# gregspangenberg/shoulder

Measured on AMD Instinct MI355X. Metric: humerus meshes/s end-to-end (all 4 landmarks), higher is better.
Workload: dtype f64 geometry + bf16 UNet

## Files before the change

shoulder_amd/csrc/k_groove.h:

```cpp
#pragma once
#include "k_stages.h"

namespace sh {

#define SH_GSLOTS (SH_GROOVE_NROWS * SH_MAXPEAK)

__global__ void k_groove_rows(const double* __restrict__ itr_cs , const double* __restrict__ prox_zs,
                              const double* __restrict__ canal_axis_ct, int row0,
                              double* __restrict__ xraw, double* __restrict__ ptheta, int* __restrict__ npk,
                              double* __restrict__ r0, int* __restrict__ err, int B) {
  __shared__ double s_bufA[SH_MPROX], s_bufB[SH_MPROX];
  double* const s_r = s_bufA; double* const s_filt = s_bufA;
  double* const s_neg = s_bufB; double* const s_roll = s_bufB;
  __shared__ int s_cand[SH_PEAK_CAP];
  __shared__ Peak s_pk[SH_PEAK_CAP];
  __shared__ int s_pass[SH_PEAK_CAP];
  __shared__ int s_ncand;
  const int M = SH_MPROX;
  const int gid = blockIdx.x, lane = threadIdx.x;
  const int b = gid / SH_GROOVE_NROWS, i = gid % SH_GROOVE_NROWS;
  const double* row = itr_cs + ((size_t)b * SH_NPROX + row0 + i) * 2 * M;
  const double* zs = prox_zs + (size_t)b * SH_NPROX + row0;
  for (int k = lane; k < M; k += 64) s_r[k] = row[M + k];
  if (lane == 0) s_ncand = 0;
// ... 155 lines not shown
    const double z_scaled = zs[i] * sc + (0.0 - zmin * sc);
    const double* ax = canal_axis_ct + 6 * b;
    double cu[3] = {ax[0] - ax[3], ax[1] - ax[4], ax[2] - ax[5]};
    const double n = norm3(cu);
    cu[0] /= n; cu[1] /= n; cu[2] /= n;
    const double z = zs[i], th = s_th[k];
    const double rad = row[M + s_pidx[k]];
    const double px = rad * cos(th), py = rad * sin(th);
    const double dx = px - cu[0] * z, dy = py - cu[1] * z;
    double* X = xraw + ((size_t)b * SH_GSLOTS + (size_t)i * SH_MAXPEAK + k) * 9;
    X[0] = rad; X[1] = near; X[2] = next; X[3] = z_scaled; X[4] = s_pk[k].prominence; X[5] = s_pk[k].width;
    X[6] = s_pk[k].width_height; X[7] = sqrt(dx * dx + dy * dy); X[8] = (double)np_ / 7.0;
    ptheta[(size_t)b * SH_GSLOTS + (size_t)i * SH_MAXPEAK + k] = th;
    for (int q = 0; q < 9; ++q) if (X[q] != X[q]) atomicCAS(&err[b], 0, SH_ERR_GEOMETRY_DEV);
  }
  if (lane == 0) npk[gid] = np_;
  (void)B;
}

__global__ void __launch_bounds__(256)
k_groove_scale(const double* __restrict__ xraw, const int* __restrict__ npk, double* __restrict__ stats, int B,
               int* __restrict__ slots_out , int* __restrict__ nslot_out ,
               float* __restrict__ proba ) {
  __shared__ double col[5][SH_GSLOTS];
  __shared__ int slot[SH_GSLOTS];
  __shared__ int P_s;
  const int b = blockIdx.x, tid = threadIdx.x;
  const double* X = xraw + (size_t)b * SH_GSLOTS * 9;
  const int* np_ = npk + (size_t)b * SH_GROOVE_NROWS;
  __shared__ int s_cnt[SH_GROOVE_NROWS];
  for (int i = tid; i < SH_GROOVE_NROWS; i += 256) s_cnt[i] = np_[i];
  __syncthreads();
  for (int i = tid; i < SH_GROOVE_NROWS; i += 256) {
    int off = 0;
    for (int j = 0; j < i; ++j) off += s_cnt[j];
    const int n = s_cnt[i];
    for (int k = 0; k < n; ++k) slot[off + k] = i * SH_MAXPEAK + k;
    if (i == SH_GROOVE_NROWS - 1) P_s = off + n;
  }
  __syncthreads();
  const int P = P_s;
  for (int p = tid; p < P; p += 256) slots_out[(size_t)b * SH_GSLOTS + p] = slot[p];
  if (tid == 0) nslot_out[b] = P;
  for (int s = tid; s < SH_GSLOTS; s += 256)
    if (s % SH_MAXPEAK >= s_cnt[s / SH_MAXPEAK]) proba[(size_t)b * SH_GSLOTS + s] = -1.0f;
  for (int f0 = 0; f0 < 9; f0 += 5) {
    const int nf = f0 + 5 <= 9 ? 5 : 9 - f0;
    for (int q = tid; q < P * nf; q += 256) { const int p = q / nf, f = q - p * nf; col[f][p] = X[(size_t)slot[p] * 9 + f0 + f]; }
    __syncthreads();
    if (tid < nf) {
      const double* c = col[tid];
      double s = 0.0;
      int p = 0;
      for (; p + 8 <= P; p += 8) {
        double t8[8];
#pragma unroll
        for (int u = 0; u < 8; ++u) t8[u] = c[p + u];
#pragma unroll
        for (int u = 0; u < 8; ++u) s += t8[u];
      }
      for (; p < P; ++p) s += c[p];
      const double mean = P ? s / (double)P : 0.0;
      double v = 0.0;
      p = 0;
      for (; p + 8 <= P; p += 8) {
        double t8[8];
#pragma unroll
        for (int u = 0; u < 8; ++u) t8[u] = c[p + u];
#pragma unroll
        for (int u = 0; u < 8; ++u) { const double d = t8[u] - mean; v += d * d; }
      }
      for (; p < P; ++p) { double d = c[p] - mean; v += d * d; }
      const double var = P ? v / (double)P : 0.0;
      const double eps_ = 2.220446049250313e-16, nn = (double)P;
      const double ub = nn * eps_ * var + (nn * mean * eps_) * (nn * mean * eps_);
      double scale = var <= ub ? 1.0 : sqrt(var);
      stats[(size_t)b * 18 + f0 + tid] = mean;
      stats[(size_t)b * 18 + 9 + f0 + tid] = scale;
    }
    __syncthreads();
  }
}

__global__ void k_rfc_pack(const int* __restrict__ feat, const float* __restrict__ thr, const int* __restrict__ ti, const int* __restrict__ fi,
                           const float* __restrict__ lw, int4* __restrict__ nodes, int N) {
  const int i = blockIdx.x * blockDim.x + threadIdx.x;
  if (i >= N) return;
  const bool leaf = ti[i] < 0;
  nodes[i] = make_int4(feat[i], __float_as_int(leaf ? lw[i] : thr[i]), ti[i], fi[i]);
}

__global__ void __launch_bounds__(64)
k_groove_rfc(const double* __restrict__ xraw, const int* __restrict__ slots , const int* __restrict__ nslot , const double* __restrict__ stats,
             const int4* __restrict__ nodes, const int* __restrict__ roots, int n_trees,
             double* __restrict__ xs , float* __restrict__ proba, int B) {
  __shared__ double sx[9][64];
  const int tid = threadIdx.x;
  constexpr int WPB = (SH_GSLOTS + 63) / 64;
  const int b = blockIdx.x / WPB, p = (blockIdx.x - b * WPB) * 64 + tid;
  if (b >= B || p >= nslot[b]) return;
  const int gid = b * SH_GSLOTS + slots[(size_t)b * SH_GSLOTS + p];
  for (int f = 0; f < 9; ++f) {
    const double v = (xraw[(size_t)gid * 9 + f] - stats[(size_t)b * 18 + f]) / stats[(size_t)b * 18 + 9 + f];
    xs[(size_t)gid * 9 + f] = v;
    sx[f][tid] = v;
  }
  double acc = 0.0;
  for (int t = 0; t < n_trees; ++t) {
    int4 nd = nodes[roots[t]];
    while (nd.z >= 0) nd = nodes[(sx[nd.x][tid] <= (double)__int_as_float(nd.y)) ? nd.z : nd.w];
    acc += (double)__int_as_float(nd.y);
  }
  proba[gid] = (float)acc;
}

#define SH_KDE_TIE 1e-9
__device__ inline double groove_kde_wg(const double* __restrict__ ptheta, const float* __restrict__ proba, double* __restrict__ bg_theta,
                                       int* __restrict__ err, int b) {
  __shared__ double sel[SH_GSLOTS];
  __shared__ double dens[1024];
  __shared__ int nsel;
  __shared__ double wv[4];
  __shared__ int wi[4];
  __shared__ double s_bg;
  int tid = threadIdx.x;
  __shared__ int s_wc[4];
  if (tid == 0) nsel = 0;
  __syncthreads();
  for (int s0 = 0; s0 < SH_GSLOTS; s0 += 256) {
    const int s = s0 + tid;
    const bool keep = s < SH_GSLOTS && proba[(size_t)b * SH_GSLOTS + s] > 0.4f;
    const double val = keep ? ptheta[(size_t)b * SH_GSLOTS + s] : 0.0;
    const unsigned long long m = __ballot(keep);
    if ((tid & 63) == 0) s_wc[tid >> 6] = __popcll(m);
    __syncthreads();
    int pos = nsel + __popcll(m & ((1ull << (tid & 63)) - 1ull));
    for (int w = 0; w < (tid >> 6); ++w) pos += s_wc[w];
    if (keep) sel[pos] = val;
    __syncthreads();
    if (tid == 0) nsel += s_wc[0] + s_wc[1] + s_wc[2] + s_wc[3];
    __syncthreads();
  }
  const int n = nsel;
  if (n == 0) { if (tid == 0) { atomicCAS(&err[b], 0, SH_ERR_GEOMETRY_DEV); bg_theta[b] = 0.0; } return 0.0; }
  double best = -1.0;
  for (int j = tid; j < 1024; j += blockDim.x) {
    double t = linspace_at(-1.0 * M_PI, M_PI, 1024, j);
    double acc = 0.0;
    for (int i = 0; i < n; ++i) {
      double d = 1.0 - fabs(t - sel[i]);
      if (d > 0.0) acc += d;
    }
    dens[j] = acc;
    best = fmax(best, acc);
  }
  for (int off = 32; off > 0; off >>= 1) best = fmax(best, __shfl_down(best, off));
  if ((tid & 63) == 0) wv[tid >> 6] = best;
  __syncthreads();
  best = wv[0];
  for (int w = 1; w < (int)(blockDim.x >> 6); ++w) best = fmax(best, wv[w]);
  const double thr = best * (1.0 - SH_KDE_TIE);
  int bi = 0x7fffffff;
  for (int j = tid; j < 1024; j += blockDim.x)
    if (dens[j] >= thr) bi = min(bi, j);
  for (int off = 32; off > 0; off >>= 1) bi = min(bi, __shfl_down(bi, off));
  if ((tid & 63) == 0) wi[tid >> 6] = bi;
  __syncthreads();
  if (tid == 0) {
    for (int w = 1; w < (int)(blockDim.x >> 6); ++w) bi = min(bi, wi[w]);
    s_bg = linspace_at(-1.0 * M_PI, M_PI, 1024, bi);
    bg_theta[b] = s_bg;
  }
  __syncthreads();
  return s_bg;
}

__device__ inline void groove_localmin_row(const double* __restrict__ itr_cs, const double* __restrict__ r0, const double* __restrict__ prox_zs,
                                           const double* __restrict__ prox_centroids, double bg, int row0, double deg_window,
                                           int* __restrict__ local_idx, double* pts_obb, int b, int i) {
  const int gid = b * SH_GROOVE_NROWS + i;
  const double* row = itr_cs + ((size_t)b * SH_NPROX + row0 + i) * 2 * SH_MPROX;
  int ivar = (int)rint(deg_window / (360.0 / (double)SH_MPROX));
  if (ivar < 1) ivar = 1;
  int loc = groove_local_min(row, r0 + (size_t)gid * SH_MPROX, SH_MPROX, bg, ivar);
  local_idx[gid] = loc;
  int k = loc < 0 ? loc + SH_MPROX : loc;
  k = k < 0 ? 0 : (k >= SH_MPROX ? SH_MPROX - 1 : k);
  double t = row[k], r = row[SH_MPROX + k];
  const double* c = prox_centroids + 2 * ((size_t)b * SH_NPROX + row0 + i);
  double* p = pts_obb + (size_t)gid * 3;
  p[0] = r * cos(t) + c[0];
  p[1] = r * sin(t) + c[1];
  p[2] = prox_zs[(size_t)b * SH_NPROX + row0 + i] + 0.0;
}

__device__ inline void groove_axis_wave(const double* pts_obb, const double* __restrict__ T_obb, double* __restrict__ axis_ct,
// ... 34 lines not shown
```

shoulder_amd/csrc/k_stages.h:

```cpp
#pragma once
#include "k_slices.h"

namespace sh {

__global__ void k_synth_batch(const float* __restrict__ tv, const int* __restrict__ tf, long long V, long long F,
                              const double* __restrict__ T, float* __restrict__ verts, int* __restrict__ faces) {
  int b = blockIdx.y;
  const double* Tb = T + 16 * b;
  for (long long i = blockIdx.x * (long long)blockDim.x + threadIdx.x; i < V; i += (long long)gridDim.x * blockDim.x) {
    double o[3];
    xform_pt(Tb, (double)tv[3 * i], (double)tv[3 * i + 1], (double)tv[3 * i + 2], o);
    float* q = verts + 3 * (V * b + i);
    q[0] = (float)o[0]; q[1] = (float)o[1]; q[2] = (float)o[2];
  }
  for (long long i = blockIdx.x * (long long)blockDim.x + threadIdx.x; i < 3 * F; i += (long long)gridDim.x * blockDim.x)
    faces[3 * F * b + i] = tf[i];
}

__global__ void k_affine_f64(const double* __restrict__ T, const double* __restrict__ in, double* __restrict__ out,
                             const long long* __restrict__ off) {
  int b = blockIdx.y;
  const double* Tb = T + 16 * b;
  long long o0 = off[b], n = off[b + 1] - o0;
  for (long long i = blockIdx.x * (long long)blockDim.x + threadIdx.x; i < n; i += (long long)gridDim.x * blockDim.x) {
// ... 19 lines not shown
  const double ox = plane[0], oy = plane[1], oz = plane[2], nx = plane[3], ny = plane[4], nz = plane[5];
  for (long long fi = blockIdx.x * (long long)blockDim.x + threadIdx.x; fi < nf; fi += (long long)gridDim.x * blockDim.x) {
    int id[3] = {faces[3 * fi], faces[3 * fi + 1], faces[3 * fi + 2]};
    double P[3][3], d[3];
    int s[3];
    for (int k = 0; k < 3; ++k) {
      for (int q = 0; q < 3; ++q) P[k][q] = (double)verts[3 * (size_t)id[k] + q];
      d[k] = ((P[k][0] - ox) * nx + (P[k][1] - oy) * ny) + (P[k][2] - oz) * nz;
      s[k] = d[k] < -SH_SECTION_TOL ? -1 : 1;
    }
    if (s[0] == s[1] && s[1] == s[2]) continue;
    int dn = 0;
    for (int j = 0; j < 3; ++j) if (s[j] == 1 && s[(j + 1) % 3] == -1) dn = j;
    int a = dn, c = (dn + 1) % 3;
    int l = id[a] < id[c] ? a : c, h = id[a] < id[c] ? c : a;
    double t = d[l] / (d[l] - d[h]);
    int slot = atomicAdd(count, 1);
    if (slot < cap)
      for (int q = 0; q < 3; ++q) out[3 * (size_t)slot + q] = P[l][q] + t * (P[h][q] - P[l][q]);
  }
}

__device__ inline double wave_kth_smallest_nonneg(const double* v, int n, int k, unsigned* hist) {
  const int lane = threadIdx.x & 63;
  unsigned long long prefix = 0, mask = 0;
  for (int shift = 56; shift >= 0; shift -= 8) {
    for (int i = lane; i < 256; i += 64) hist[i] = 0;
    __syncthreads();
    for (int i = lane; i < n; i += 64) {
      const unsigned long long u = (unsigned long long)__double_as_longlong(v[i]);
      if ((u & mask) == prefix) atomicAdd(&hist[(u >> shift) & 255], 1u);
    }
    __syncthreads();
    const unsigned c0 = hist[4 * lane], c1 = hist[4 * lane + 1], c2 = hist[4 * lane + 2], c3 = hist[4 * lane + 3];
    const unsigned tot = c0 + c1 + c2 + c3;
    unsigned incl = tot;
    for (int off = 1; off < 64; off <<= 1) { unsigned o = __shfl_up(incl, off); if (lane >= off) incl += o; }
    const unsigned excl = incl - tot;
    if ((unsigned)k >= excl && (unsigned)k < incl) {
      unsigned r = (unsigned)k - excl, bin = 4 * lane;
      if (r >= c0) { r -= c0; ++bin; if (r >= c1) { r -= c1; ++bin; if (r >= c2) { r -= c2; ++bin; } } }
      hist[256] = bin; hist[257] = r;
    }
    __syncthreads();
    prefix |= (unsigned long long)hist[256] << shift;
    mask |= 0xffull << shift;
    k = (int)hist[257];
    __syncthreads();
  }
  return __longlong_as_double((long long)prefix);
}

template <bool BIG>
__global__ void __launch_bounds__(64)
k_neck(const double* __restrict__ areas, const double* __restrict__ zs, double* __restrict__ neck_z, int* __restrict__ neck_index, int B,
       double c0, double c1, double* __restrict__ gscratch ) {
  __shared__ double Ks[BIG ? 1 : SH_CPD_MAXN * SH_CPD_MAXN];
  __shared__ unsigned hist[258];
  int b = blockIdx.x, lane = threadIdx.x;
  int a, e;
  cutoff_range(SH_NFULL, c0, c1, &a, &e);
  int n = e - a;
  if (!BIG && n > SH_CPD_MAXN) n = SH_CPD_MAXN;
  double* K;
  if (BIG) K = gscratch + (size_t)b * SH_NFULL * SH_NFULL; else K = Ks;
  const double* x = areas + (size_t)b * SH_NFULL + a;
  for (int i = 0; i < n; ++i) {
    const int base = i * n - i * (i + 1) / 2 - (i + 1);
    for (int j = i + 1 + lane; j < n; j += 64) { double d = x[i] - x[j]; K[base + j] = d * d; }
  }
  __syncthreads();
  const int np_ = n * (n - 1) / 2;
  double med;
  __threadfence_block();
  if (np_ & 1) med = wave_kth_smallest_nonneg(K, np_, np_ / 2, hist);
  else { double lo = wave_kth_smallest_nonneg(K, np_, np_ / 2 - 1, hist); double hi = wave_kth_smallest_nonneg(K, np_, np_ / 2, hist); med = (lo + hi) / 2.0; }
  const double gamma = (med == 0.0) ? 1.0 : 1.0 / med;
  __syncthreads();
  for (int q = lane; q < n * n; q += 64) K[q] = cpd_kernel(x[q / n], x[q % n], gamma);
  __syncthreads();
  double best = 1e300;
  int bt = 0x7fffffff;
  for (int t = 2 + lane; t <= n - 2; t += 64) {
    double cst = cpd_cost(K, n, t);
    if (cst < best) { best = cst; bt = t; }
  }
  for (int off = 32; off > 0; off >>= 1) {
    double ob = __shfl_down(best, off);
    int ot = __shfl_down(bt, off);
    if (ob < best || (ob == best && ot < bt)) { best = ob; bt = ot; }
  }
  if (lane == 0) {
    neck_index[b] = bt;
    neck_z[b] = zs[(size_t)b * SH_NFULL + a + bt];
  }
}

__global__ void k_prox_obb(const double* __restrict__ area_scan , const double* __restrict__ scan_zs, const double* __restrict__ T_pre,
                           double* __restrict__ T_obb, int* __restrict__ flipped, double* __restrict__ cutoff , int* __restrict__ cutoff_idx ,
                           int* __restrict__ err, int B) {
  const int b = blockIdx.x * blockDim.x + threadIdx.x;
  if (b >= B) return;
  const double* A = area_scan + (size_t)b * SH_NPSCAN;
  int k = 0;
  for (int j = 1; j < SH_NPSCAN; ++j) if (A[j] > A[k]) k = j;
  const bool flip = scan_zs[(size_t)b * SH_NPSCAN + k] < 0;
  double ar[SH_NPSCAN], tmp[2 * SH_NPSCAN];
  for (int j = 0; j < SH_NPSCAN; ++j) ar[j] = flip ? A[SH_NPSCAN - 1 - j] : A[j];
  int lo, hi;
  if (prox_canal_range(ar, SH_NPSCAN, tmp, &lo, &hi) < 1) atomicCAS(&err[b], 0, SH_ERR_GEOMETRY_DEV);
  cutoff_idx[2 * b] = lo; cutoff_idx[2 * b + 1] = hi;
  cutoff[2 * b] = (double)lo / (double)SH_NPSCAN;
  cutoff[2 * b + 1] = (double)hi / (double)SH_NPSCAN;
  flipped[b] = flip ? 1 : 0;
  const double* Tp = T_pre + 16 * b;
  double* To = T_obb + 16 * b;
  for (int q = 0; q < 16; ++q) To[q] = Tp[q];
  if (flip) for (int q = 0; q < 4; ++q) { To[q] = -Tp[q]; To[8 + q] = -Tp[8 + q]; }
}

__device__ inline double wave_sum(double v) {
  for (int off = 32; off > 0; off >>= 1) v += __shfl_down(v, off);
  return __shfl(v, 0);
}

__device__ inline void wave_line_fit(const double* p, int n, int stride, double* mean, double* dir) {
  int lane = threadIdx.x & 63;
  double s[3] = {0, 0, 0};
  for (int i = lane; i < n; i += 64) { s[0] += p[(size_t)i * stride]; s[1] += p[(size_t)i * stride + 1]; s[2] += p[(size_t)i * stride + 2]; }
  for (int k = 0; k < 3; ++k) mean[k] = wave_sum(s[k]) / (double)n;
  double c[6] = {0, 0, 0, 0, 0, 0};
  for (int i = lane; i < n; i += 64) {
    double x = p[(size_t)i * stride] - mean[0], y = p[(size_t)i * stride + 1] - mean[1], z = p[(size_t)i * stride + 2] - mean[2];
    c[0] += x * x; c[1] += x * y; c[2] += x * z; c[3] += y * y; c[4] += y * z; c[5] += z * z;
  }
  for (int k = 0; k < 6; ++k) c[k] = wave_sum(c[k]);
  double C[9] = {c[0], c[1], c[2], c[1], c[3], c[4], c[2], c[4], c[5]};
  dominant_eigvec3(C, dir);
}

#define SH_CANAL_MAXPTS SH_NFULL
__global__ void k_canal(const double* __restrict__ centroids, const double* __restrict__ zs, const double* __restrict__ zb,
                        const double* __restrict__ T_obb, double c0, double c1, const double* __restrict__ cut ,
                        double* __restrict__ pts_obb, double* __restrict__ axis_obb, double* __restrict__ axis_ct, int* __restrict__ err) {
  int b = blockIdx.x, lane = threadIdx.x;
  if (cut) { c0 = cut[2 * b]; c1 = cut[2 * b + 1]; }
  int a, e;
  cutoff_range(SH_NFULL, c0, c1, &a, &e);
  int n = e - a;
  if (n > SH_CANAL_MAXPTS) n = SH_CANAL_MAXPTS;
  if (n < 2) { if (lane == 0) { atomicCAS(&err[b], 0, SH_ERR_GEOMETRY_DEV); for (int k = 0; k < 6; ++k) { axis_obb[6 * b + k] = 0; axis_ct[6 * b + k] = 0; } } return; }
  double* P = pts_obb + (size_t)b * SH_CANAL_MAXPTS * 3;
  for (int i = lane; i < n; i += 64) {
    P[3 * i] = centroids[2 * ((size_t)b * SH_NFULL + a + i)];
    P[3 * i + 1] = centroids[2 * ((size_t)b * SH_NFULL + a + i) + 1];
    P[3 * i + 2] = zs[(size_t)b * SH_NFULL + a + i];
  }
  __syncthreads();
  double mean[3], d[3];
  wave_line_fit(P, n, 3, mean, d);
  if (lane == 0) {
    if (d[2] < 0) { d[0] = -d[0]; d[1] = -d[1]; d[2] = -d[2]; }
    double z_length = fabs(zb[2 * b]) + fabs(zb[2 * b + 1]);
    double half = (z_length * ((c0 + c1) / 2.0)) / 2.0;
    double* A = axis_obb + 6 * b;
    for (int k = 0; k < 3; ++k) { A[k] = mean[k] + d[k] * half; A[3 + k] = mean[k] - d[k] * half; }
    double Ti[16];
// ... 8 lines not shown
```

shoulder_amd/csrc/sh_ctx.h:

```cpp
#pragma once
#include "../../include/shoulder_hip.h"

#include <hip/hip_runtime.h>

#include <algorithm>
#include <atomic>
#include <chrono>
#include <cmath>
#include <condition_variable>
#include <cstddef>
#include <cstdio>
#include <cstring>
#include <deque>
#include <functional>
#include <initializer_list>
#include <map>
#include <memory>
#include <mutex>
#include <string>
#include <thread>
#include <tuple>
#include <vector>

#include "sh_demand.h"
// ... 48 lines not shown
  int open_mode = SH_OPEN_ERROR;
  double open_gap = SH_OPEN_GAP_DEFAULT;
  int open_stats_run = SH_OPEN_ERROR;
  int end_cap = SH_ENDCAP;
  unsigned long long obb_gen = ~0ull;
  sh::HullCap hcap = {SH_HV, SH_HF, SH_HE};
  int obb_sil_need = 0;
  bool obb_nf_over = false;
  bool hull_force_host = false;
  std::vector<float> h_verts;
  bool h_verts_valid = false;
  float* h_kept = nullptr; long long h_kept_cap = 0;
  int* h_nkept = nullptr; int h_nkept_cap = 0;
  struct HullPts { const float* src = nullptr;
                   std::vector<long long> off;
                   std::vector<int> cnt; };
  HullPts hull_in;
  long long* h_koff = nullptr; int h_koff_cap = 0;
  struct StageSide {
    bool active = false, from_stl = false;
    int B = 0; long long sumV = 0, sumF = 0, maxV = 0, maxF = 0;
    std::vector<long long> voff, foff;
    void* h_src = nullptr; size_t h_src_cap = 0;
    int* h_flag = nullptr;
    size_t h_flag_cap = 0;
    float* h_kept = nullptr; long long h_kept_cap = 0;
    long long* h_koff = nullptr; int h_koff_cap = 0;
    HullPts pts;
    hipEvent_t ready_ev = nullptr;
    std::mutex m; std::condition_variable cv; bool meta_ready = true; int meta_rc = 0; std::string meta_err;
  } stg;
  int b0 = 0, Bwin = 0;
  struct HullStage { double* hv = nullptr; double* nr = nullptr; int* ed = nullptr; int* cnt = nullptr; int cap = 0; hipEvent_t ev = nullptr; bool used = false;
                     int pv = 4096, pf = 8192, pe = 12288; };
  HullStage hstage[2];
  int hslot = 0;
  struct Prepared {
    std::thread th; bool active = false; int slot = 0, B = 0, rc = SH_OK, bad_mesh = -1; unsigned long long gen = 0;
    double d2h_ms = 0, hull_ms = 0; std::string err;
    bool uploaded = false;
    bool staged = false;
  } prep;
  hipEvent_t obb_done_ev = nullptr;
  struct Ticket { hipEvent_t ev = nullptr; char* status = nullptr ; int cap = 0, B = 0; bool pending = false; sh_landmarks* host_out = nullptr;
                  uint32_t mask = 0; sh_landmarks* out_arg = nullptr; bool dev_hull = false; unsigned long long gen = 0; size_t rec = sizeof(sh_landmarks); int rows = 0; };
  Ticket tickets[2];
  int t_head = 0, t_tail = 0, n_pending = 0;
  hipStream_t out_stream = nullptr;
  bool overlap = false;
  unsigned long long batch_gen = 0;
  uint32_t rec_mask = 0;
  unsigned long long rec_gen = ~0ull, resect_gen = ~0ull;
  int resect_P = 0;
  unsigned long long canal_gen = ~0ull;
  sh_canal_grid canal_grid = {0.0, 0.0, 0, 0};
  unsigned long long resect_seq = 0, canal_seq = 0;
  unsigned long long seat_resect_seq = ~0ull, stem_resect_seq = ~0ull, stem_canal_seq = ~0ull;
  int seat_K = 0, stem_K = 0;
  hipStream_t copy_stream = nullptr;
  hipEvent_t stl_counted_ev = nullptr;
  hipStream_t side_stream = nullptr;
  hipEvent_t side_fork_ev = nullptr, side_join_ev = nullptr;
  struct Switches {
    int window = 0;
    bool obb_prune = true;
    bool slice_merge = true;
    bool hull_prefilter = true;
    bool debug = false;
  } sw;
  struct Unet {
    bool reference = false;
    bool turn = false;
    hipEvent_t done_ev = nullptr;
    int num_cus = 0;
    int ticket_next = 0;
    std::map<std::tuple<int, int, int>, std::pair<int, int>> tk_tabs;
    int tk_tab_used = 0;
    bool zero_page_ready = false;
    bool packtab_ready = false;
    bool packed_x3 = false;
    int packed_kind = -1;
  } unet;
  bool packed_rfc = false;
  int timing = 0;
  std::vector<std::tuple<std::string, hipEvent_t, hipEvent_t>> pending;
  std::map<std::string, KTimer> timers;
};

#define HIPCHK(ctx, call)                                                                   \
  do {                                                                                      \
    hipError_t e_ = (call);                                                                 \
    if (e_ != hipSuccess) {                                                                 \
      (ctx)->err = std::string(#call) + ": " + hipGetErrorString(e_);                       \
      return SH_ERR_HIP;                                                                    \
    }                                                                                       \
  } while (0)

#define HIPCHK_TXT(errtxt, call) do { hipError_t e_ = (call); if (e_ != hipSuccess) { *(errtxt) = std::string(#call) + ": " + hipGetErrorString(e_); return SH_ERR_HIP; } } while (0)

struct WindowScope {
  sh_ctx* c; int b0, Bwin;
  WindowScope(sh_ctx* c_, int nb0, int nBwin) : c(c_), b0(c_->b0), Bwin(c_->Bwin) { c->b0 = nb0; c->Bwin = nBwin; }
  ~WindowScope() { c->b0 = b0; c->Bwin = Bwin; }
  WindowScope(const WindowScope&) = delete; WindowScope& operator=(const WindowScope&) = delete;
};

struct StreamScope {
  sh_ctx* c; hipStream_t saved;
  StreamScope(sh_ctx* c_, hipStream_t s) : c(c_), saved(c_->stream) { c->stream = s; }
  ~StreamScope() { c->stream = saved; }
  StreamScope(const StreamScope&) = delete; StreamScope& operator=(const StreamScope&) = delete;
};

static inline void params_changed(sh_ctx* c) { c->unet.packed_kind = -1; c->unet.packed_x3 = false; c->packed_rfc = false; }

static inline int fail(sh_ctx* c, int code, const std::string& msg) {
  if (c) c->err = msg;
  return code;
}

static inline int ensure(sh_ctx* c, const char* name, size_t bytes, int elem, void** out = nullptr) {
  Buf& b = c->bufs[name];
  if (b.bytes < bytes || b.p == nullptr) {
    if (b.p) (void)hipFree(b.p);
    b.p = nullptr;
    hipError_t e = hipMalloc(&b.p, bytes ? bytes : 16);
    if (e != hipSuccess) {
      c->err = std::string("hipMalloc(") + name + "): " + hipGetErrorString(e);
      b.bytes = 0;
      return SH_ERR_NOMEM;
    }
    b.bytes = bytes;
  }
  b.elem = elem;
  if (out) *out = b.p;
  return SH_OK;
}

template <typename T>
static inline T* buf(sh_ctx* c, const char* name) {
  auto it = c->bufs.find(name);
  if (it == c->bufs.end() || !it->second.p) return nullptr;
  return (T*)((char*)it->second.p + (size_t)c->b0 * it->second.per_mesh);
}

struct HullRec { double *hv, *normals; int *edges, *nv, *nf, *ne; };
static inline HullRec hull_rec(sh_ctx* c) {
  return {buf<double>(c, "hull.hv"), buf<double>(c, "hull.normals"), buf<int>(c, "hull.edges"), buf<int>(c, "hull.nv"), buf<int>(c, "hull.nf"), buf<int>(c, "hull.ne")};
}

#define ENS_(name, bytes, elem, per_mesh_)                                          \
  do {                                                                              \
    if ((rc = ensure(c, name, (size_t)(bytes), elem)) != SH_OK) return rc;          \
    c->bufs[name].per_mesh = (per_mesh_);                                           \
  } while (0)
#define ENS(name, bytes, elem) ENS_(name, bytes, elem, (size_t)(bytes) / (size_t)c->B)
#define ENS_SHARED(name, bytes, elem) ENS_(name, bytes, elem, 0)
template <typename T> constexpr int elem_of() { return sizeof(T) <= 8 ? (int)sizeof(T) : 1; }

static inline bool timed_launch(const sh_ctx* c, const char* name) {
  return c->timing == 1 || (c->timing == 2 && name[0] == 'u' && name[1] == 'n' && name[2] == 'e' && name[3] == 't' && name[4] == '.');
}

#define LAUNCH_FN(ctx, name, call)                                                           \
  do {                                                                                      \
    hipEvent_t e0_ = nullptr, e1_ = nullptr;                                                \
// ... 41 lines not shown
```

shoulder_amd/csrc/sh_scalar.h:

```cpp
#pragma once
#include "sh_common.h"

namespace sh {

#define SH_CPD_MAXN 64
SH_HD double kth_smallest(double* a, int n, int k) {
  int lo = 0, hi = n - 1;
  while (lo < hi) {
    double p = a[(lo + hi) >> 1];
    int i = lo, j = hi;
    while (i <= j) {
      while (a[i] < p) ++i;
      while (a[j] > p) --j;
      if (i <= j) { double t = a[i]; a[i] = a[j]; a[j] = t; ++i; --j; }
    }
    if (k <= j) hi = j; else if (k >= i) lo = i; else break;
  }
  return a[k];
}

SH_HD double cpd_gamma(const double* x, int n, double* pd) {
  int np_ = n * (n - 1) / 2;
  int c = 0;
  for (int i = 0; i < n; ++i)
    for (int j = i + 1; j < n; ++j) { double d = x[i] - x[j]; pd[c++] = d * d; }
  double med;
  if (np_ & 1) med = kth_smallest(pd, np_, np_ / 2);
  else { double a = kth_smallest(pd, np_, np_ / 2 - 1); double b = kth_smallest(pd, np_, np_ / 2); med = (a + b) / 2.0; }
  return (med == 0.0) ? 1.0 : 1.0 / med;
}
SH_HD double cpd_kernel(double xi, double xj, double gamma) {
  double d = xi - xj;
  double v = d * d * gamma;
  v = v < 1e-2 ? 1e-2 : (v > 1e2 ? 1e2 : v);
  return exp(-v);
}
SH_HD double cpd_cost(const double* K, int n, int t) {
  double d0 = 0, s0 = 0, d1 = 0, s1 = 0;
  for (int i = 0; i < t; ++i) { d0 += K[i * n + i]; for (int j = 0; j < t; ++j) s0 += K[i * n + j]; }
  for (int i = t; i < n; ++i) { d1 += K[i * n + i]; for (int j = t; j < n; ++j) s1 += K[i * n + j]; }
  return (d0 - s0 / (double)t) + (d1 - s1 / (double)(n - t));
}
SH_HD int cpd_one_bkp(const double* x, int n, double* scratch) {
  const int min_size = 2;
  double* K = scratch + n * (n - 1) / 2;
  double gamma = cpd_gamma(x, n, scratch);
  for (int i = 0; i < n; ++i)
    for (int j = 0; j < n; ++j) K[i * n + j] = cpd_kernel(x[i], x[j], gamma);
  int best_t = -1;
  double best = 1e300;
  for (int t = min_size; t <= n - min_size; ++t) {
    double cst = cpd_cost(K, n, t);
    if (cst < best) { best = cst; best_t = t; }
  }
  return best_t;
}

SH_HD int prox_canal_range(const double* area, int n, double* tmp, int* lo, int* hi) {
  double* sm = tmp;
  double* g = tmp + n;
  for (int i = 1; i + 1 < n; ++i) sm[i] = ((area[i - 1] + area[i]) + area[i + 1]) / 3.0;
  sm[0] = ((5.0 * area[0] + 2.0 * area[1]) - area[2]) / 6.0;
  sm[n - 1] = ((5.0 * area[n - 1] + 2.0 * area[n - 2]) - area[n - 3]) / 6.0;
  g[0] = sm[1] - sm[0];
  g[n - 1] = sm[n - 1] - sm[n - 2];
  for (int i = 1; i + 1 < n; ++i) g[i] = (sm[i + 1] - sm[i - 1]) / 2.0;
  int best_a = 0, best_len = 0, a = -1;
  for (int i = 0; i <= n; ++i) {
    const bool in = i < n && g[i] < 10.0;
    if (in && a < 0) a = i;
    if (!in && a >= 0) { if (i - a > best_len) { best_len = i - a; best_a = a; } a = -1; }
  }
  *lo = best_a; *hi = best_len > 0 ? best_a + best_len - 1 : best_a;
  return best_len;
}

SH_HD double circle_residual_at(const double* xy, int n, double cx, double cy, double* g, double* H) {
  double sr = 0, sux = 0, suy = 0;
  for (int i = 0; i < n; ++i) {
    double dx = xy[2 * i] - cx, dy = xy[2 * i + 1] - cy;
    double r = sqrt(dx * dx + dy * dy);
    sr += r; sux += dx / r; suy += dy / r;
  }
  double rm = sr / n, mux = sux / n, muy = suy / n;
  double f2 = 0;
  if (g) { g[0] = g[1] = 0; H[0] = H[1] = H[2] = 0; }
  for (int i = 0; i < n; ++i) {
    double dx = xy[2 * i] - cx, dy = xy[2 * i + 1] - cy;
    double r = sqrt(dx * dx + dy * dy);
    double f = r - rm;
    f2 += f * f;
    if (g) {
      double jx = -(dx / r - mux), jy = -(dy / r - muy);
      g[0] += jx * f; g[1] += jy * f;
      H[0] += jx * jx; H[1] += jx * jy; H[2] += jy * jy;
    }
  }
  return f2;
}

SH_HD double circle_fit_residual(const double* xy, int n, double* cx_out = nullptr, double* cy_out = nullptr) {
  double cx = 0, cy = 0;
  for (int i = 0; i < n; ++i) { cx += xy[2 * i]; cy += xy[2 * i + 1]; }
  cx /= n; cy /= n;
  double lam = 1e-3, g[2], H[3];
  double f2 = circle_residual_at(xy, n, cx, cy, g, H);
  for (int it = 0; it < 200; ++it) {
    double a = H[0] * (1 + lam), b = H[1], d = H[2] * (1 + lam);
    double det = a * d - b * b;
    if (det == 0) break;
    double sx = -(d * g[0] - b * g[1]) / det, sy = -(-b * g[0] + a * g[1]) / det;
    double g2[2], H2[3];
    double f2n = circle_residual_at(xy, n, cx + sx, cy + sy, g2, H2);
    if (f2n <= f2) {
      cx += sx; cy += sy;
      bool done = (fabs(sx) + fabs(sy)) < 1e-13 * (1.0 + fabs(cx) + fabs(cy));
      f2 = f2n; g[0] = g2[0]; g[1] = g2[1]; H[0] = H2[0]; H[1] = H2[1]; H[2] = H2[2];
      lam *= 0.2;
      if (done) break;
    } else {
      lam *= 10.0;
      if (lam > 1e12) break;
    }
// ... 758 lines not shown
```

shoulder_amd/csrc/shoulder_hip.hip:

```cpp
#include "sh_ctx.h"

#include "k_slices.h"
#include "k_ovf.h"
#include "k_open.h"
#include "k_stages.h"
#include "k_groove.h"
#include "k_anp.h"
#include "k_stl.h"
#include "k_clip.h"
#include "k_resect.h"
#include "k_headfit.h"
#include "k_seat.h"
#include "k_stem.h"
#include "k_plan.h"
#include "k_te.h"
#include "k_obb.h"
#include "sh_hull.h"

#include <sched.h>

using namespace sh;

struct FillList { void* p[6]; unsigned long long n[6]; unsigned v[6]; };
__global__ void k_fill_list(FillList L) {
// ... 1333 lines not shown
  if (!c->obb_done_ev) HIPCHK(c, hipEventCreateWithFlags(&c->obb_done_ev, hipEventDisableTiming));
  HIPCHK(c, hipEventRecord(c->obb_done_ev, c->stream));
  if (c->params.bone_kind == SH_BONE_PROXIMAL) {
    dim3 gv((unsigned)std::min<long long>((c->maxV + 255) / 256, 1024), (unsigned)B);
    LAUNCH(c, "k_transform_verts", k_transform_verts, gv, dim3(256), v.verts, v.voff, v.obb_T_pre, v.verts_obb, v.zb_enc);
    w->bounds_cleared = false;
    int rc2;
    if ((rc2 = run_slice_set(c, v, SPEC_POBB)) != SH_OK) return rc2;
    LAUNCH(c, "k_prox_obb", k_prox_obb, dim3((B + 63) / 64), dim3(64), v.set[SET_POBB].area_total, v.set[SET_POBB].zs, v.obb_T_pre,
           v.obb_transform, v.flipped, v.pobb_cutoff, v.pobb_cutoff_idx, v.err, B);
    c->obb_injected = true;
    return SH_OK;
  }
  dim3 g((unsigned)std::min<long long>((c->maxF + 255) / 256, 1024), (unsigned)B);
  LAUNCH(c, "k_obb_end_points", k_obb_end_points, g, dim3(256), v.verts, v.faces, v.voff, v.foff, v.obb_T_pre, v.obb_zb_pre, v.obb_endpts, v.obb_endcnt, c->end_cap);
  LAUNCH(c, "k_obb_ends", k_obb_ends, dim3(B), dim3(128), v.obb_endpts, v.obb_endcnt, v.obb_T_pre, v.obb_resid, v.obb_transform, v.flipped, v.err, B, c->end_cap,
         v.ovf_ctr + SH_CTR_END_NEED);
  c->obb_injected = true;
  return SH_OK;
}

static int run_te_rows(sh_ctx* c, const WinView& v) {
  const int B = v.B;
  const SliceSetView& distal = v.set[SET_DISTAL];
  OvfPools OP; OvfSet OS;
  { int orc; if ((orc = ovf_pools(c, &OP)) != SH_OK || (orc = ovf_set(c, "distal", SH_NDIST, &OS)) != SH_OK) return orc; }
  LAUNCH(c, "k_te_rows", k_te_rows<SH_SMALLSEG>, dim3(B * SH_TE_NROWS), dim3(64), distal.ring, distal.ring_n, v.te_rects, B, (const long long*)OS.roff);
  LAUNCH(c, "k_te_rows_large", k_te_rows<SH_MAXSEG>, dim3(B * SH_TE_NROWS), dim3(64), distal.ring, distal.ring_n, v.te_rects, B, (const long long*)OS.roff);
  if (c->ovf_none_gen != c->batch_gen) LAUNCH(c, "k_te_rows_huge", k_te_rows_huge, dim3(64), dim3(64), OP, OS, (const int*)distal.ring_n, v.te_rects);
  LAUNCH(c, "k_te_ends", k_te_ends, dim3(B), dim3(64), distal.ring, distal.ring_n, v.te_rects, distal.zs, v.obb_transform, v.te_ends_ct, v.te_row, v.err, B, OP, OS);
  return SH_OK;
}

static int stage_frame(sh_ctx* c, const WinView& v, uint32_t mask, const WinState& w) {
  const int B = v.B;
  if (!w.bounds_cleared && (mask & (SH_STAGE_OBB | SH_STAGE_FULL | SH_STAGE_ANP)))
    FILL(c, {v.zb_enc, (size_t)B * 16, 0xFF}, {v.anp_mm_enc, (size_t)B * 16, 0xFF});
  if (mask & (SH_STAGE_OBB | SH_STAGE_FULL)) {
    dim3 g((unsigned)std::min<long long>((c->maxV + 255) / 256, 1024), (unsigned)B);
    LAUNCH(c, "k_transform_verts", k_transform_verts, g, dim3(256), v.verts, v.voff, v.obb_transform, v.verts_obb, v.zb_enc);
    if (!(mask & SH_STAGE_FULL))
      LAUNCH(c, "k_decode_bounds", k_decode_bounds, dim3((2 * B + 63) / 64), dim3(64), v.zb_enc, v.z_bounds, B);
  }
  return SH_OK;
}

static int fork_side(sh_ctx* c) {
  if (!c->side_stream) HIPCHK(c, hipStreamCreateWithFlags(&c->side_stream, hipStreamNonBlocking));
  if (!c->side_fork_ev) { HIPCHK(c, hipEventCreateWithFlags(&c->side_fork_ev, hipEventDisableTiming)); HIPCHK(c, hipEventCreateWithFlags(&c->side_join_ev, hipEventDisableTiming)); }
  HIPCHK(c, hipEventRecord(c->side_fork_ev, c->stream));
  HIPCHK(c, hipStreamWaitEvent(c->side_stream, c->side_fork_ev, 0));
  return SH_OK;
}

static int stage_distal(sh_ctx* c, const WinView& v, uint32_t mask, bool merged, bool side, WinState* w) {
  int rc;
  if (side && (rc = fork_side(c)) != SH_OK) return rc;
  {
    StreamScope on(c, side ? c->side_stream : c->stream);
    rc = merged ? SH_OK : run_slice_set(c, v, spec_distal(false));
    const bool te_inline = !side && (mask & SH_STAGE_ANP);
    if (rc == SH_OK && (side || te_inline) && (mask & SH_STAGE_TE)) { rc = run_te_rows(c, v); w->te_rows_done = rc == SH_OK; }
  }
  if (side && rc == SH_OK) { HIPCHK(c, hipEventRecord(c->side_join_ev, c->side_stream)); w->side_pending = true; }
  return rc;
}

static int stage_neck(sh_ctx* c, const WinView& v, bool with_prox) {
  const bool prox = c->params.bone_kind == SH_BONE_PROXIMAL;
  LAUNCH(c, "k_neck", prox ? k_neck<true> : k_neck<false>, dim3(v.B), dim3(64), v.set[SET_FULL].areas, v.set[SET_FULL].zs, v.neck_z, v.neck_index, v.B,
         prox ? 0.2 : 0.70, 0.99, prox ? v.neck_gram : (double*)nullptr);
  if (!with_prox) return run_slice_set(c, v, SPEC_NECKC);
  const SliceSpec sp[2] = {SPEC_NECKC, SPEC_PROX};
  return run_slice_sets(c, v, sp, 2);
}

static int stage_canal(sh_ctx* c, const WinView& v) {
  LAUNCH(c, "k_canal", k_canal, dim3(v.B), dim3(64), v.set[SET_FULL].centroids, v.set[SET_FULL].zs, v.z_bounds, v.obb_transform, c->params.canal_cutoff[0],
         c->params.canal_cutoff[1], c->params.bone_kind == SH_BONE_PROXIMAL ? v.pobb_cutoff : (const double*)nullptr,
         v.canal_points_obb, v.canal_axis_obb, v.canal_axis_ct, v.err);
  return SH_OK;
}

static int stage_groove(sh_ctx* c, const WinView& v, uint32_t mask) {
  const int B = v.B;
  int rc;
  if (!c->have_rfc) return fail(c, SH_ERR_STATE, "sh_run: groove stage needs sh_load_rfc first");
  int ga, gb;
  cutoff_range(SH_NPROX, c->params.groove_cutoff[0], c->params.groove_cutoff[1], &ga, &gb);
  if (!(mask & SH_STAGE_PROXIMAL) && !(c->rs_gen == c->batch_gen && (c->rs_all || (ga >= c->rs_cs_lo && gb <= c->rs_cs_hi))))
    return fail(c, SH_ERR_STATE, "sh_run: SH_STAGE_GROOVE without SH_STAGE_PROXIMAL, and the proximal slices of this batch were not made for this groove_cutoff (run SH_STAGE_PROXIMAL again)");
  const char* pp = buf<char>(c, "params") + c->unet_floats * 4;
  const size_t N = c->h_feat.size();
  const int* feat = (const int*)pp; const float* thr = (const float*)(pp + N * 4); const int* ti = (const int*)(pp + N * 8);
  const int* fi = (const int*)(pp + N * 12); const float* lw = (const float*)(pp + N * 16); const int* roots = (const int*)(pp + N * 20);
  const double* prox_zs = v.set[SET_PROX].zs;
  LAUNCH(c, "k_groove_rows", k_groove_rows, dim3(B * SH_GROOVE_NROWS), dim3(64), v.prox_itr_centered_start, prox_zs, v.canal_axis_ct, ga, v.groove_xraw,
         v.groove_ptheta, v.groove_npk, v.groove_r0, v.err, B);
  LAUNCH(c, "k_groove_scale", k_groove_scale, dim3(B), dim3(256), v.groove_xraw, v.groove_npk, v.groove_stats, B, v.groove_slots, v.groove_nslot, v.groove_proba);
  if ((rc = ensure(c, "rfc.nodes", N * 16, 4)) != SH_OK) return rc;
  int4* nodes = (int4*)c->bufs["rfc.nodes"].p;
  if (!c->packed_rfc) {
    LAUNCH(c, "k_rfc_pack", k_rfc_pack, dim3((unsigned)((N + 255) / 256)), dim3(256), feat, thr, ti, fi, lw, nodes, (int)N);
    c->packed_rfc = true;
  }
  LAUNCH(c, "k_groove_rfc", k_groove_rfc, dim3((unsigned)(B * ((SH_GSLOTS + 63) / 64))), dim3(64), v.groove_xraw, v.groove_slots, v.groove_nslot,
         v.groove_stats, nodes, roots, c->rfc_trees, v.groove_xs, v.groove_proba, B);
  LAUNCH(c, "k_groove_tail", k_groove_tail, dim3(B), dim3(256), v.groove_ptheta, v.groove_proba, v.groove_bg_theta, v.err,
         v.prox_itr_centered_start, v.groove_r0, prox_zs, v.set[SET_PROX].centroids, ga, c->params.groove_deg_window,
         v.groove_local_idx, v.groove_points_obb, v.obb_transform, v.groove_axis_ct, v.groove_points_ct);
  return SH_OK;
}

static int stage_anp(sh_ctx* c, const WinView& v) {
  const int B = v.B;
  int rc;
  if (!c->have_unet) return fail(c, SH_ERR_STATE, "sh_run: anatomic-neck stage needs sh_load_unet first");
  LAUNCH(c, "k_anp_rows", k_anp_rows, dim3(B * SH_ANP_ROWS), dim3(64), v.prox_itr_start, v.groove_bg_theta, v.anp_raw, v.anp_t01, v.anp_roll, B,
         v.anp_mm_enc);
  const bool scale_in_net = plan_level0_fused(c->params.unet_dtype, c->unet.reference, c->unet_base, c->unet_depth, SH_ANP_ROWS, SH_MPROX);
  if (!scale_in_net || c->keep_products) LAUNCH(c, "k_anp_scale", k_anp_scale, dim3(64, B), dim3(256), v.anp_raw, v.anp_mm_enc, v.anp_image);
  if ((rc = unet_turn_enter(c)) != SH_OK) return rc;
  rc = unet_dispatch(c, {v.anp_image, scale_in_net ? v.anp_raw : nullptr, scale_in_net ? v.anp_mm_enc : nullptr, v.anp_logits}, B, SH_ANP_ROWS, SH_MPROX);
  (void)unet_turn_leave(c);
  if (rc != SH_OK) return rc;
  const double* prox_zs = v.set[SET_PROX].zs;
  LAUNCH(c, "k_anp_edge_count", k_anp_edge_count, dim3(SH_ANP_ROWS / 8, B), dim3(512), v.anp_logits, v.anp_rowcnt, v.anp_maskbits);
  LAUNCH(c, "k_anp_edges", k_anp_edges, dim3(SH_ANP_ROWS / 8, B), dim3(512), v.anp_maskbits, v.anp_raw, v.anp_t01, v.anp_roll, prox_zs, v.anp_rowcnt,
         v.anp_points_obb, v.anp_counts, v.err);
  LAUNCH(c, "k_anp_plane", k_anp_plane, dim3(B), dim3(256), v.anp_points_obb, v.anp_counts, v.anp_plane, v.err, v.anp_ray_t);
  LAUNCH(c, "k_rays_hit", k_rays_hit, dim3(SH_RAY_CHUNKS, B), dim3(256), v.verts_obb, v.faces, v.voff, v.foff, v.anp_plane, v.anp_ray_t);
  return SH_OK;
}

static int stage_tail(sh_ctx* c, const WinView& v, uint32_t mask) {
  const int B = v.B;
  const bool prox = c->params.bone_kind == SH_BONE_PROXIMAL;
  const uint32_t need = SH_STAGE_GROOVE | SH_STAGE_ANP | SH_STAGE_CSYS | (prox ? 0u : (uint32_t)SH_STAGE_TE);
  const bool metrics = (mask & need) == need;
  if (metrics)
    LAUNCH(c, "k_sphere_partial", k_sphere_partial, dim3(SH_SPH_PARTS, B), dim3(256), v.anp_maskbits, v.anp_raw, v.anp_t01, v.anp_roll, v.set[SET_PROX].zs,
           v.anp_plane, v.metrics_partial);
  PackArgs A{};
  A.lm = v.landmarks; A.T_obb = v.obb_transform; A.zb = v.z_bounds; A.neck_z = v.neck_z;
  A.neck_index = v.neck_index; A.flipped = v.flipped; A.canal_axis_ct = v.canal_axis_ct; A.te_axis_ct = v.te_axis_ct;
  A.groove_axis_ct = v.groove_axis_ct; A.bg_theta = v.groove_bg_theta; A.groove_pts_ct = v.groove_points_ct;
  A.plane = v.anp_plane; A.axes_obb = v.anp_axes_obb; A.anp_pts_obb = v.anp_points_obb; A.anp_counts = v.anp_counts;
  A.err = v.err; A.mask = mask; A.B = B; A.bone_kind = (int)c->params.bone_kind;
  A.canal_cut = prox ? v.pobb_cutoff : (const double*)nullptr;
  A.cc0 = c->params.canal_cutoff[0]; A.cc1 = c->params.canal_cutoff[1];
  A.ray_t = v.anp_ray_t; A.te_ends_ct = v.te_ends_ct; A.sphere_partial = v.metrics_partial; A.metrics = metrics ? 1 : 0;
  LAUNCH(c, "k_tail", k_tail, dim3(B), dim3(256), A);
  return SH_OK;
}

static int stage_apply(sh_ctx* c, const WinView& v) {
  dim3 g((unsigned)std::min<long long>((c->maxV + 255) / 256, 1024), (unsigned)v.B);
  LAUNCH(c, "k_apply_csys", k_apply_csys, g, dim3(256), v.landmarks, v.verts, v.voff, v.verts_csys);
  return SH_OK;
}

static int run_window(sh_ctx* c, uint32_t mask, int prepared_slot, int redo_nf = 0) {
  auto has = [mask](uint32_t stages) { return (mask & stages) != 0; };
  int rc;
  WinView v = win_view(c);
  WinState w;
  if (has(SH_STAGE_OBB) && (rc = run_obb(c, v, &w, prepared_slot, redo_nf)) != SH_OK) return rc;
  if ((rc = stage_frame(c, v, mask, w)) != SH_OK) return rc;
  const bool transformed = has(SH_STAGE_OBB | SH_STAGE_FULL);
  const bool merge_env = c->sw.slice_merge;
  const bool can_fork = has(SH_STAGE_DISTAL) && c->ovf_none_gen == c->batch_gen && c->timing != 1 && redo_nf == 0;
  const bool side = can_fork && v.B <= 16;
  const bool merge_fd = merge_env && has(SH_STAGE_FULL) && has(SH_STAGE_DISTAL) && !side;
  if (merge_fd) {
    const SliceSpec sp[2] = {spec_full(transformed), spec_distal(transformed)};
    if ((rc = run_slice_sets(c, v, sp, 2)) != SH_OK) return rc;
  } else if (has(SH_STAGE_FULL)) {
    if ((rc = run_slice_set(c, v, spec_full(transformed))) != SH_OK) return rc;
  }
  if (has(SH_STAGE_DISTAL) && (rc = stage_distal(c, v, mask, merge_fd, side, &w)) != SH_OK) return rc;
  const bool merge_np = merge_env && has(SH_STAGE_NECK) && has(SH_STAGE_PROXIMAL);
  if (has(SH_STAGE_NECK) && (rc = stage_neck(c, v, merge_np)) != SH_OK) return rc;
  if (has(SH_STAGE_CANAL) && (rc = stage_canal(c, v)) != SH_OK) return rc;
  if (has(SH_STAGE_PROXIMAL) && !merge_np && (rc = run_slice_set(c, v, SPEC_PROX)) != SH_OK) return rc;
  if (has(SH_STAGE_GROOVE) && (rc = stage_groove(c, v, mask)) != SH_OK) return rc;
  if (has(SH_STAGE_ANP) && (rc = stage_anp(c, v)) != SH_OK) return rc;
  if (w.side_pending) { HIPCHK(c, hipStreamWaitEvent(c->stream, c->side_join_ev, 0)); w.side_pending = false; }
  if (has(SH_STAGE_TE) && !w.te_rows_done && (rc = run_te_rows(c, v)) != SH_OK) return rc;
  if ((rc = stage_tail(c, v, mask)) != SH_OK) return rc;
  if (has(SH_STAGE_APPLY) && (rc = stage_apply(c, v)) != SH_OK) return rc;
// ... 805 lines not shown
```

Before: 9278.

## Stage random-forest trees in LDS with BFS layout and double buffering

Random-forest inference now reorders each tree breadth-first on the host so its nodes sit contiguously with tree-relative child indices. It runs 256-thread blocks that stage each tree (up to 1024 nodes) in shared memory, double-buffered so the next tree's load overlaps the current walk. This replaces scattered global-memory node fetches with LDS reads, at the cost of a per-tree block barrier and more LDS per block. Separately, the neck CPD cost loop now uses an unrolled blocked row-sum helper.

```diff
diff --git a/shoulder_amd/csrc/k_groove.h b/shoulder_amd/csrc/k_groove.h
--- a/shoulder_amd/csrc/k_groove.h
+++ b/shoulder_amd/csrc/k_groove.h
@@ -261,36 +261,75 @@
   }
 }
 
-__global__ void k_rfc_pack(const int* __restrict__ feat, const float* __restrict__ thr, const int* __restrict__ ti, const int* __restrict__ fi,
-                           const float* __restrict__ lw, int4* __restrict__ nodes, int N) {
-  const int i = blockIdx.x * blockDim.x + threadIdx.x;
-  if (i >= N) return;
-  const bool leaf = ti[i] < 0;
-  nodes[i] = make_int4(feat[i], __float_as_int(leaf ? lw[i] : thr[i]), ti[i], fi[i]);
-}
-
-__global__ void __launch_bounds__(64)
+#define SH_RFC_LDS_NODES 1024
+__global__ void k_rfc_pack(const int* __restrict__ feat, const float* __restrict__ thr, const float* __restrict__ lw,
+                           const int* __restrict__ src, const int* __restrict__ lt, const int* __restrict__ lf, int4* __restrict__ nodes, int Np) {
+  const int q = blockIdx.x * blockDim.x + threadIdx.x;
+  if (q >= Np) return;
+  const int i = src[q];
+  const bool leaf = lt[q] < 0;
+  nodes[q] = make_int4(feat[i], __float_as_int(leaf ? lw[i] : thr[i]), lt[q], lf[q]);
+}
+
+typedef int rfc_node_t __attribute__((ext_vector_type(4)));
+
+template <typename NodePtr>
+__device__ inline double rfc_walk_tree(NodePtr T, const double (*sx)[256], int tid) {
+  int4 nd = T[0];
+  asm volatile("" : "+v"(nd.x), "+v"(nd.y), "+v"(nd.z), "+v"(nd.w));
+  while (nd.z >= 0) {
+    nd = T[(sx[nd.x][tid] <= (double)__int_as_float(nd.y)) ? nd.z : nd.w];
+    asm volatile("" : "+v"(nd.x), "+v"(nd.y), "+v"(nd.z), "+v"(nd.w));
+  }
+  return (double)__int_as_float(nd.y);
+}
+
+__global__ void __launch_bounds__(256)
 k_groove_rfc(const double* __restrict__ xraw, const int* __restrict__ slots , const int* __restrict__ nslot , const double* __restrict__ stats,
-             const int4* __restrict__ nodes, const int* __restrict__ roots, int n_trees,
+             const int4* __restrict__ nodes, const int2* __restrict__ trees , int n_trees,
              double* __restrict__ xs , float* __restrict__ proba, int B) {
-  __shared__ double sx[9][64];
+  __shared__ double sx[9][256];
+  __shared__ int4 s_tree[2][SH_RFC_LDS_NODES];
+  constexpr int NR = SH_RFC_LDS_NODES / 256;
   const int tid = threadIdx.x;
-  constexpr int WPB = (SH_GSLOTS + 63) / 64;
-  const int b = blockIdx.x / WPB, p = (blockIdx.x - b * WPB) * 64 + tid;
-  if (b >= B || p >= nslot[b]) return;
-  const int gid = b * SH_GSLOTS + slots[(size_t)b * SH_GSLOTS + p];
-  for (int f = 0; f < 9; ++f) {
-    const double v = (xraw[(size_t)gid * 9 + f] - stats[(size_t)b * 18 + f]) / stats[(size_t)b * 18 + 9 + f];
-    xs[(size_t)gid * 9 + f] = v;
-    sx[f][tid] = v;
-  }
+  constexpr int WPB = (SH_GSLOTS + 255) / 256;
+  const int b = blockIdx.x / WPB, p0 = (blockIdx.x - b * WPB) * 256;
+  if (b >= B) return;
+  const int ns = nslot[b];
+  if (p0 >= ns) return;
+  const bool live = p0 + tid < ns;
+  int gid = 0;
+  if (live) {
+    gid = b * SH_GSLOTS + slots[(size_t)b * SH_GSLOTS + p0 + tid];
+    for (int f = 0; f < 9; ++f) {
+      const double v = (xraw[(size_t)gid * 9 + f] - stats[(size_t)b * 18 + f]) / stats[(size_t)b * 18 + 9 + f];
+      xs[(size_t)gid * 9 + f] = v;
+      sx[f][tid] = v;
+    }
+  }
+  int2 cur = trees[0];
+  if (cur.y <= SH_RFC_LDS_NODES)
+    for (int k = tid; k < cur.y; k += 256) s_tree[0][k] = nodes[cur.x + k];
+  __syncthreads();
   double acc = 0.0;
   for (int t = 0; t < n_trees; ++t) {
-    int4 nd = nodes[roots[t]];
-    while (nd.z >= 0) nd = nodes[(sx[nd.x][tid] <= (double)__int_as_float(nd.y)) ? nd.z : nd.w];
-    acc += (double)__int_as_float(nd.y);
-  }
-  proba[gid] = (float)acc;
+    const bool more = t + 1 < n_trees;
+    const int2 nxt = more ? trees[t + 1] : make_int2(0, 0);
+    const bool stage = more && nxt.y <= SH_RFC_LDS_NODES;
+    rfc_node_t r[NR] = {};
+    if (stage) {
+#pragma unroll
+      for (int u = 0; u < NR; ++u) if (tid + 256 * u < nxt.y) r[u] = ((const rfc_node_t*)nodes)[nxt.x + tid + 256 * u];
+    }
+    if (live) acc += cur.y <= SH_RFC_LDS_NODES ? rfc_walk_tree((const int4*)s_tree[t & 1], sx, tid) : rfc_walk_tree(nodes + cur.x, sx, tid);
+    if (stage) {
+#pragma unroll
+      for (int u = 0; u < NR; ++u) if (tid + 256 * u < nxt.y) ((rfc_node_t*)s_tree[(t + 1) & 1])[tid + 256 * u] = r[u];
+    }
+    __syncthreads();
+    cur = nxt;
+  }
+  if (live) proba[gid] = (float)acc;
 }
 
 #define SH_KDE_TIE 1e-9
diff --git a/shoulder_amd/csrc/k_stages.h b/shoulder_amd/csrc/k_stages.h
--- a/shoulder_amd/csrc/k_stages.h
+++ b/shoulder_amd/csrc/k_stages.h
@@ -125,7 +125,7 @@
   double best = 1e300;
   int bt = 0x7fffffff;
   for (int t = 2 + lane; t <= n - 2; t += 64) {
-    double cst = cpd_cost(K, n, t);
+    double cst = cpd_cost_blocked(K, n, t);
     if (cst < best) { best = cst; bt = t; }
   }
   for (int off = 32; off > 0; off >>= 1) {
diff --git a/shoulder_amd/csrc/sh_ctx.h b/shoulder_amd/csrc/sh_ctx.h
--- a/shoulder_amd/csrc/sh_ctx.h
+++ b/shoulder_amd/csrc/sh_ctx.h
@@ -154,6 +154,7 @@
     int packed_kind = -1;
   } unet;
   bool packed_rfc = false;
+  std::vector<int32_t> h_rfc_layout;
   int timing = 0;
   std::vector<std::tuple<std::string, hipEvent_t, hipEvent_t>> pending;
   std::map<std::string, KTimer> timers;
diff --git a/shoulder_amd/csrc/sh_scalar.h b/shoulder_amd/csrc/sh_scalar.h
--- a/shoulder_amd/csrc/sh_scalar.h
+++ b/shoulder_amd/csrc/sh_scalar.h
@@ -39,6 +39,26 @@
   double d0 = 0, s0 = 0, d1 = 0, s1 = 0;
   for (int i = 0; i < t; ++i) { d0 += K[i * n + i]; for (int j = 0; j < t; ++j) s0 += K[i * n + j]; }
   for (int i = t; i < n; ++i) { d1 += K[i * n + i]; for (int j = t; j < n; ++j) s1 += K[i * n + j]; }
+  return (d0 - s0 / (double)t) + (d1 - s1 / (double)(n - t));
+}
+SH_HD double cpd_row_sum(const double* r, int m, double s) {
+  int j = 0;
+  for (; j + 8 <= m; j += 8) {
+    double t8[8];
+    for (int u = 0; u < 8; ++u) t8[u] = r[j + u];
+    for (int u = 0; u < 8; ++u) s += t8[u];
+  }
+  if (j < m) {
+    double t8[8];
+    for (int u = 0; u < 7; ++u) t8[u] = j + u < m ? r[j + u] : 0.0;
+    for (int u = 0; u < 7; ++u) if (j + u < m) s += t8[u];
+  }
+  return s;
+}
+SH_HD double cpd_cost_blocked(const double* K, int n, int t) {
+  double d0 = 0, s0 = 0, d1 = 0, s1 = 0;
+  for (int i = 0; i < t; ++i) { d0 += K[i * n + i]; s0 = cpd_row_sum(K + i * n, t, s0); }
+  for (int i = t; i < n; ++i) { d1 += K[i * n + i]; s1 = cpd_row_sum(K + i * n + t, n - t, s1); }
   return (d0 - s0 / (double)t) + (d1 - s1 / (double)(n - t));
 }
 SH_HD int cpd_one_bkp(const double* x, int n, double* scratch) {
diff --git a/shoulder_amd/csrc/shoulder_hip.hip b/shoulder_amd/csrc/shoulder_hip.hip
--- a/shoulder_amd/csrc/shoulder_hip.hip
+++ b/shoulder_amd/csrc/shoulder_hip.hip
@@ -1439,6 +1439,31 @@
   return SH_OK;
 }
 
+static int rfc_tree_layout(const std::vector<int32_t>& ti, const std::vector<int32_t>& fi, const std::vector<int32_t>& roots, std::vector<int32_t>* out) {
+  const size_t N = ti.size(), T = roots.size();
+  std::vector<int32_t> src, lt, lf, tree;
+  src.reserve(N); lt.reserve(N); lf.reserve(N); tree.reserve(2 * T);
+  for (size_t t = 0; t < T; ++t) {
+    const size_t first = src.size();
+    src.push_back(roots[t]);
+    for (size_t q = first; q < src.size(); ++q) {
+      const int i = src[q];
+      if (ti[i] >= 0) {
+        lt.push_back((int32_t)(src.size() - first)); src.push_back(ti[i]);
+        lf.push_back((int32_t)(src.size() - first)); src.push_back(fi[i]);
+      } else { lt.push_back(-1); lf.push_back(-1); }
+    }
+    tree.push_back((int32_t)first); tree.push_back((int32_t)(src.size() - first));
+  }
+  const int Np = (int)src.size();
+  out->clear();
+  out->insert(out->end(), tree.begin(), tree.end());
+  out->insert(out->end(), src.begin(), src.end());
+  out->insert(out->end(), lt.begin(), lt.end());
+  out->insert(out->end(), lf.begin(), lf.end());
+  return Np;
+}
+
 static int stage_groove(sh_ctx* c, const WinView& v, uint32_t mask) {
   const int B = v.B;
   int rc;
@@ -1449,20 +1474,25 @@
     return fail(c, SH_ERR_STATE, "sh_run: SH_STAGE_GROOVE without SH_STAGE_PROXIMAL, and the proximal slices of this batch were not made for this groove_cutoff (run SH_STAGE_PROXIMAL again)");
   const char* pp = buf<char>(c, "params") + c->unet_floats * 4;
   const size_t N = c->h_feat.size();
-  const int* feat = (const int*)pp; const float* thr = (const float*)(pp + N * 4); const int* ti = (const int*)(pp + N * 8);
-  const int* fi = (const int*)(pp + N * 12); const float* lw = (const float*)(pp + N * 16); const int* roots = (const int*)(pp + N * 20);
+  const int* feat = (const int*)pp; const float* thr = (const float*)(pp + N * 4); const float* lw = (const float*)(pp + N * 16);
   const double* prox_zs = v.set[SET_PROX].zs;
   LAUNCH(c, "k_groove_rows", k_groove_rows, dim3(B * SH_GROOVE_NROWS), dim3(64), v.prox_itr_centered_start, prox_zs, v.canal_axis_ct, ga, v.groove_xraw,
          v.groove_ptheta, v.groove_npk, v.groove_r0, v.err, B);
   LAUNCH(c, "k_groove_scale", k_groove_scale, dim3(B), dim3(256), v.groove_xraw, v.groove_npk, v.groove_stats, B, v.groove_slots, v.groove_nslot, v.groove_proba);
+  const size_t T = c->h_roots.size();
   if ((rc = ensure(c, "rfc.nodes", N * 16, 4)) != SH_OK) return rc;
+  if ((rc = ensure(c, "rfc.layout", (3 * N + 2 * T) * 4, 4)) != SH_OK) return rc;
   int4* nodes = (int4*)c->bufs["rfc.nodes"].p;
+  int* layout = (int*)c->bufs["rfc.layout"].p;
   if (!c->packed_rfc) {
-    LAUNCH(c, "k_rfc_pack", k_rfc_pack, dim3((unsigned)((N + 255) / 256)), dim3(256), feat, thr, ti, fi, lw, nodes, (int)N);
+    const int Np = rfc_tree_layout(c->h_ti, c->h_fi, c->h_roots, &c->h_rfc_layout);
+    HIPCHK(c, hipMemcpyAsync(layout, c->h_rfc_layout.data(), c->h_rfc_layout.size() * 4, hipMemcpyHostToDevice, c->stream));
+    const int* src = layout + 2 * T;
+    LAUNCH(c, "k_rfc_pack", k_rfc_pack, dim3((unsigned)((Np + 255) / 256)), dim3(256), feat, thr, lw, src, src + Np, src + 2 * (size_t)Np, nodes, Np);
     c->packed_rfc = true;
   }
-  LAUNCH(c, "k_groove_rfc", k_groove_rfc, dim3((unsigned)(B * ((SH_GSLOTS + 63) / 64))), dim3(64), v.groove_xraw, v.groove_slots, v.groove_nslot,
-         v.groove_stats, nodes, roots, c->rfc_trees, v.groove_xs, v.groove_proba, B);
+  LAUNCH(c, "k_groove_rfc", k_groove_rfc, dim3((unsigned)(B * ((SH_GSLOTS + 255) / 256))), dim3(256), v.groove_xraw, v.groove_slots, v.groove_nslot,
+         v.groove_stats, nodes, (const int2*)layout, c->rfc_trees, v.groove_xs, v.groove_proba, B);
   LAUNCH(c, "k_groove_tail", k_groove_tail, dim3(B), dim3(256), v.groove_ptheta, v.groove_proba, v.groove_bg_theta, v.err,
          v.prox_itr_centered_start, v.groove_r0, prox_zs, v.set[SET_PROX].centroids, ga, c->params.groove_deg_window,
          v.groove_local_idx, v.groove_points_obb, v.obb_transform, v.groove_axis_ct, v.groove_points_ct);
```

Measured after the change: 9170. 1.2% lower.
